# TianyiFranklinWang/MIRROR

Measured on AMD Instinct MI355X. Metric: SSL samples/sec (slide+RNA pairs), higher is better.
Workload: dtype bf16; 1 GPU; BASELINE c2: B=16/GPU x [4096 patch tokens x 1024-d] + [2048 genes], D=512, RNA depth 6 / 8 heads, train mode, local-batch InfoNCE; precision_policy=bf16, per_gpu_batch=16, global_batch=16, parallelism=dp1, grad_bucket_dtype=f32, step_launch=hip_graph

## Files before the change

### include/mirror_hip.h

```cpp
#ifndef MIRROR_HIP_H
#define MIRROR_HIP_H
#include <stdint.h>

#ifdef __cplusplus
extern "C" {
#endif

#define MH_OK 0
#define MH_EINVAL (-1)
#define MH_EUNSUP (-2)
#define MH_EHIP (-3)

#define MH_F32 0
#define MH_BF16 1

#define MH_ACT_NONE 0
#define MH_ACT_RELU 1
#define MH_ACT_GELU 2

typedef void* mh_stream;

const char* mh_last_error(void);
int mh_version(void);
int mh_exp_build(void);
// ... 166 lines not shown
int mh_eye_minus(const float* P, float* T, float d, int BH, int m, mh_stream s);

int mh_seq_finish(void* seq, const float* cls, int B, int N, int add, int D, int dt, mh_stream s);
int mh_seq_finish_bwd(void* dseq, float* dcls, int B, int N, int add, int D, int dt, mh_stream s);
int mh_ppeg_merge(const float* w7, const float* w5, const float* w3, const float* b7, const float* b5,
                  const float* b3, float* merged, float* bsum, int D, mh_stream s);
int mh_ppeg_fwd(const void* x, void* y, const float* merged, const float* bsum, int B, int S, int D,
                int flip, int dt_x, int dt_y, mh_stream s);
int mh_ppeg_wgrad(const void* x, const void* dout, float* dmerged, float* dbsum, int B, int S, int D,
                  int dt_x, int dt_o, mh_stream s);
int mh_ppeg_bwd(const float* x, const float* dy, const float* merged, float* dx, float* dmerged, float* dbsum, int B, int S,
                int D, void* drop_out, float* drop_db, float p, uint64_t seed, uint64_t offset, const uint64_t* dev_base,
                mh_stream s);
int mh_ppeg_grad_scatter(const float* dmerged, const float* dbsum, float* dw7, float* dw5, float* dw3, float* db7,
                         float* db5, float* db3, int D, mh_stream s);

int mh_rank_mask(const float* noise, float* mask, int B, int N, int len_keep, mh_stream s);
int mh_mask_apply_fwd(const void* x, void* y, const float* mask, const float* token, const float* pos, int B, int T, int D,
                      int first, int token_scalar, int dt_x, int dt_y, mh_stream s);
int mh_mask_apply_bwd_dbias_ok(const void* dy, const void* dx, const float* dpos, int D, int dt_dy, int dt_dx);
int mh_mask_apply_bwd(const void* dy, void* dx, const float* mask, float* dtoken, float* dpos, int B, int T, int D,
                      int first, int token_scalar, int dt_dy, int dt_dx, float* dbias, mh_stream s);

typedef struct {
    int32_t B, D, Hh, H;
    float eps, p_drop;
    uint64_t seed, offset;
    const uint64_t* dev_base;
    const void *w_qkv, *w_proj, *w_fc1, *w_fc2;
    const void *wt_qkv, *wt_proj, *wt_fc1, *wt_fc2;
    const float *b_qkv, *b_proj, *b_fc1, *b_fc2;
    const float *g1, *be1, *g2, *be2;
    const float* x;
    float* y;
    float* stats;
    void* qkv;
    float* attn;
    void* o;
    float* x1;
    void* u;
    void* f;
    const float* dy;
    float* dx;
    float *dw_qkv, *dw_proj, *dw_fc1, *dw_fc2, *db_qkv, *db_proj, *db_fc1, *db_fc2, *dg1, *dbe1, *dg2, *dbe2;
    void* scratch;
} mh_rna_block;
// ... 206 lines not shown
```

### mirror_amd/_lib.py

```python
from __future__ import annotations

import ctypes as C
import os

_HERE = os.path.dirname(os.path.abspath(__file__))
LIB_PATH = os.environ.get("MIRROR_HIP_LIB") or os.path.join(_HERE, "lib", "libmirror_hip.so")

MH_F32, MH_BF16 = 0, 1
ACT_NONE, ACT_RELU, ACT_GELU = 0, 1, 2


class GemmEpi(C.Structure):
    _fields_ = [
        ("kind", C.c_int32), ("resid", C.c_void_p),
        ("p", C.c_float), ("seed", C.c_uint64), ("offset", C.c_uint64), ("dev_base", C.c_void_p),
        ("mask", C.c_void_p), ("token", C.c_void_p), ("pos", C.c_void_p),
        ("rows_per_batch", C.c_int32), ("first", C.c_int32),
        ("tgt", C.c_void_p), ("tgt_bs", C.c_int64), ("sq", C.c_void_p),
    ]


class SkinnyWgradItem(C.Structure):
    _fields_ = [("dy", C.c_void_p), ("lddy", C.c_int64), ("x", C.c_void_p), ("ldx", C.c_int64), ("dw", C.c_void_p), ("lddw", C.c_int64),
                ("db", C.c_void_p), ("M", C.c_int32), ("N", C.c_int32), ("K", C.c_int32), ("dt_dy", C.c_int32), ("dt_x", C.c_int32)]
# ... 98 lines not shown
    "mh_eye_minus": [P, P, F, I, I],
    "mh_pinv_chain_prep": [P, P, P, P, P, I, I],
    "mh_pinv_chain_pack": [P, P, I, I],
    "mh_pinv_chain_fwd": [P, P, P, I, I, I, P, P, I],
    "mh_nys_sim2": [P, P, P, P, P, I, I, I, I, F, L, P],
    "mh_nys_dz_dav": [P, P, P, P, P, P, I, I, I],
    "mh_pinv_chain_bwd": [P, P, P, P, P, P, I, I, I],
    "mh_nys_attn1_fwd": [P, P, P, P, P, P, P, I, I, I, I, I, F, I, L, P],
    "mh_nys_attn1_fwd_q8": [P, P, P, P, P, I, I, I, I, I, F, I, P, P, P, F, P, P],
    "mh_nys_attn3_fwd": [P, P, P, P, P, L, P, P, I, I, I, I, I, F, L, P, P],
    "mh_nys_attn1_bwd": [P, P, P, P, P, P, P, P, P, P, P, P, I, I, I, I, I, F, L],
    "mh_nys_attn3_bwd": [P, P, P, P, P, P, P, P, P, P, I, I, I, I, I, F, L],
    "mh_nys_cls_attn": [P, P, P, P, P, P, P, I, I, I, I, I, I, F, L, I, I],
    "mh_seq_finish": [P, P, I, I, I, I, I],
    "mh_seq_finish_bwd": [P, P, I, I, I, I, I],
    "mh_ppeg_merge": [P, P, P, P, P, P, P, P, I],
    "mh_ppeg_fwd": [P, P, P, P, I, I, I, I, I, I],
    "mh_ppeg_wgrad": [P, P, P, P, I, I, I, I, I],
    "mh_ppeg_bwd": [P, P, P, P, P, P, I, I, I, P, P, F, U64, U64, P],
    "mh_ppeg_grad_scatter": [P, P, P, P, P, P, P, P, I],
    "mh_rank_mask": [P, P, I, I, I],
    "mh_mask_apply_fwd": [P, P, P, P, P, I, I, I, I, I, I, I],
    "mh_mask_apply_bwd": [P, P, P, P, P, I, I, I, I, I, I, I, P],
    "mh_headattn_fwd": [P, P, P, I, I, I, I],
    "mh_headattn_bwd": [P, P, P, P, I, I, I, I],
    "mh_add": [P, P, P, L, I, I, I],
    "mh_lm_merge": [P, P, P, L, I, L, I],
    "mh_cast": [P, P, L, I, I],
    "mh_gelu_fwd": [P, P, L, I, I],
    "mh_gelu_bwd": [P, P, P, L, I, I, I],
    "mh_relu_bwd": [P, P, P, L, I, L, L, L, I, I, I],
    "mh_dropout": [P, P, L, F, U64, U64, P, I, I],
    "mh_noise_draws": [P, L, L, U64, U64, P],
    "mh_dropout_add": [P, P, P, L, F, U64, U64, P, I],
    "mh_dropout_lite": [P, P, P, L, F, U64, U64, P, I, I],
    "mh_timestamp": [P],
    "mh_dropout_lite_colsum": [P, P, L, I, F, U64, U64, P, P],
    "mh_colsum": [P, P, L, I, L, I],
    "mh_l2norm_fwd": [P, P, P, I, I, L, F, I, I],
    "mh_l2norm_bwd": [P, P, P, P, I, I, L, F, I, I, I, I],
    "mh_exp_fwd": [P, P, L],
    "mh_exp_bwd": [P, P, P, L, I],
    "mh_reparam_fwd": [P, P, P, P, L],
    "mh_reparam_bwd": [P, P, P, P, P, P, P, L],
    "mh_ce_rows_fwd": [P, L, P, F, I, I, I, F, P, P, P],
    "mh_ce_rows_bwd": [P, L, P, F, P, P, I, F, P, P, I, I, I],
# ... 160 lines not shown
```

### mirror_amd/csrc/elementwise.hip

```cpp
#include "common.h"

#define EW_GRID(n) dim3((unsigned)min((long)mh_cdiv((n), 256), 16384L))
#define EW_LOOP(i, n) for (long i = (long)blockIdx.x * 256 + threadIdx.x; i < (n); i += (long)gridDim.x * 256)

template <typename TA, typename TB, typename TY>
__global__ __launch_bounds__(256) void add_kernel(const TA* a, const TB* b, TY* y, long n) {
    EW_LOOP(i, n) stf(y + i, ldf(a + i) + ldf(b + i));
}
template <typename TX, typename TY>
__global__ __launch_bounds__(256) void cast_kernel(const TX* x, TY* y, long n) {
    EW_LOOP(i, n) stf(y + i, ldf(x + i));
}
template <typename TX, typename TY>
__global__ __launch_bounds__(256) void gelu_fwd_kernel(const TX* x, TY* y, long n) {
    EW_LOOP(i, n) stf(y + i, gelu_f(ldf(x + i)));
}
template <typename TX, typename TDY, typename TDX>
__global__ __launch_bounds__(256) void gelu_bwd_kernel(const TX* x, const TDY* dy, TDX* dx, long n) {
    EW_LOOP(i, n) stf(dx + i, ldf(dy + i) * gelu_grad_f(ldf(x + i)));
}
template <typename TY, typename TDY, typename TDX>
__global__ __launch_bounds__(256) void relu_bwd_kernel(const TY* y, const TDY* dy, TDX* dx, long npb, long y_bs, long dy_bs, long dx_bs) {
    const long b = blockIdx.y;
    EW_LOOP(i, npb) stf(dx + b * dx_bs + i, ldf(y + b * y_bs + i) > 0.f ? ldf(dy + b * dy_bs + i) : 0.f);
// ... 442 lines not shown
extern "C" int mh_colsum(const void* x, float* out, int64_t rows, int cols, int64_t ld, int dt, mh_stream s) {
    if (rows == 0 || cols == 0) return MH_OK;
    if (dt == MH_F32 && cols % 4 == 0 && ld % 4 == 0 && ((uintptr_t)x & 15) == 0 && rows >= 32) {
        dim3 gv(mh_cdiv(cols / 4, 64), (unsigned)min((long)mh_cdiv(rows, 32), 64L));
        hipLaunchKernelGGL(colsum_f32_vec_kernel, gv, dim3(256), 0, (hipStream_t)s, (const float*)x, out, (long)rows, cols, (long)ld);
        MH_LAUNCH_CHECK("mh_colsum");
        return MH_OK;
    }
    if (dt == MH_BF16 && cols % 8 == 0 && ld % 8 == 0 && ((uintptr_t)x & 15) == 0 && rows >= 1024) {
        const int cb = mh_cdiv(cols, 512);
        long nb = max(1L, 512L / cb);
        long band = (mh_cdiv(rows, nb) + 31) / 32 * 32;
        dim3 gv(cb, mh_cdiv(rows, band));
        hipLaunchKernelGGL(colsum_bf16_vec_kernel, gv, dim3(256), 0, (hipStream_t)s, (const bf16_t*)x, out, (long)rows, cols, (long)ld, band);
        MH_LAUNCH_CHECK("mh_colsum");
        return MH_OK;
    }
    dim3 grid(mh_cdiv(cols, 64), mh_cdiv(rows, CS_BAND));
    MH_DISPATCH_DT(dt, T, hipLaunchKernelGGL((colsum_kernel<T>), grid, dim3(256), 0, (hipStream_t)s, (const T*)x, out, (long)rows, cols, (long)ld));
    MH_LAUNCH_CHECK("mh_colsum");
    return MH_OK;
}

__global__ __launch_bounds__(1024) void rank_mask_kernel(const float* __restrict__ noise, float* __restrict__ mask, int N, int P, int len_keep) {
    extern __shared__ __attribute__((aligned(16))) unsigned long long keys[];
    const long b = blockIdx.x;
    const float* nb = noise + b * N;
    for (int j = threadIdx.x; j < P; j += 1024) {
        unsigned long long k = ~0ull;
        if (j < N) {
            unsigned u = __float_as_uint(nb[j]);
            u ^= (u >> 31) ? 0xffffffffu : 0x80000000u;
            k = ((unsigned long long)u << 32) | (unsigned)j;
        }
        keys[j] = k;
    }
    __syncthreads();
    for (int k = 2; k <= P; k <<= 1)
        for (int j = k >> 1; j > 0; j >>= 1) {
            for (int t = threadIdx.x; t < (P >> 1); t += 1024) {
                const int lo = ((t & ~(j - 1)) << 1) | (t & (j - 1)), hi = lo | j;
                const unsigned long long a = keys[lo], c = keys[hi];
                const bool up = (lo & k) == 0;
                if ((a > c) == up) { keys[lo] = c; keys[hi] = a; }
            }
            __syncthreads();
        }
    for (int j = threadIdx.x; j < N; j += 1024) mask[b * N + (unsigned)(keys[j] & 0xffffffffu)] = j >= len_keep ? 1.f : 0.f;
}

extern "C" int mh_rank_mask(const float* noise, float* mask, int B, int N, int len_keep, mh_stream s) {
    MH_REQUIRE(N >= 1 && N <= 16384, "mh_rank_mask: N=%d unsupported (max 16384)", N);
    if (B == 0) return MH_OK;
    int P = 2;
    while (P < N) P <<= 1;
    static const bool big = [] {
        return hipFuncSetAttribute(reinterpret_cast<const void*>(rank_mask_kernel), hipFuncAttributeMaxDynamicSharedMemorySize, 16384 * 8) == hipSuccess;
    }();
    MH_REQUIRE(big || P * 8 <= 65536, "mh_rank_mask: %d bytes of LDS refused", P * 8);
    hipLaunchKernelGGL(rank_mask_kernel, dim3(B), dim3(1024), (size_t)P * sizeof(unsigned long long), (hipStream_t)s, noise, mask, N, P, len_keep);
    MH_LAUNCH_CHECK("mh_rank_mask");
    return MH_OK;
}

template <typename T, typename TY>
__global__ __launch_bounds__(256) void mask_apply_fwd_kernel(const T* x, TY* y, const float* __restrict__ mask,
                                                             const float* __restrict__ token, const float* __restrict__ pos, int B, int Tn,
                                                             int D, int first, int token_scalar) {
    const long total = (long)B * Tn * D;
    EW_LOOP(idx, total) {
        const int c = idx % D;
        const long bt = idx / D;
        const int t = bt % Tn;
        const long b = bt / Tn;
        float v = ldf(x + idx);
        if (t >= first && mask[b * (Tn - first) + (t - first)] != 0.f) v = token[token_scalar ? 0 : c];
        stf(y + idx, v + pos[(long)t * D + c]);
    }
}

typedef float mf_f4 __attribute__((ext_vector_type(4)));
template <typename TX>
__global__ __launch_bounds__(256) void mask_apply_fwd_vec_kernel(const TX* x, float* y, const float* __restrict__ mask,
                                                                 const float* __restrict__ token, const float* __restrict__ pos, int B,
// ... 24 lines not shown
    if (c < D) {
        for (int t = t0 + slice; t < t1; t += 4) {
            float sp = 0.f;
            for (int b = 0; b < B; b++) {
                const long at = ((long)b * Tn + t) * D + c;
                const float g = ldf(dy + at);
                sp += g;
                const bool msk = t >= first && mask[(long)b * (Tn - first) + (t - first)] != 0.f;
                if (msk) st += g;
                stf(dx + at, msk ? 0.f : g);
            }
            dpos[(long)t * D + c] += sp;
        }
    }
    red[slice][lane] = st;
    __syncthreads();
    if (slice == 0 && c < D) {
        const float tot = red[0][lane] + red[1][lane] + red[2][lane] + red[3][lane];
        if (tot != 0.f) atomicAdd(dtoken + (token_scalar ? 0 : c), tot);
    }
}

typedef float mb_f4 __attribute__((ext_vector_type(4)));
template <typename TDX>
__global__ __launch_bounds__(256) void mask_apply_bwd_vec_kernel(const float* dy, TDX* dx, const float* __restrict__ mask,
                                                                 float* __restrict__ dtoken, float* __restrict__ dpos, int B, int Tn, int D,
                                                                 int first, int token_scalar, int band, float* __restrict__ dbias) {
    __shared__ mb_f4 red[4][64];
    __shared__ mb_f4 reda[4][64];
    const int lane = threadIdx.x & 63, wave = threadIdx.x >> 6;
    const int c = blockIdx.x * 256 + 4 * lane;
    const int t0 = blockIdx.y * band, t1 = min(Tn, t0 + band);
    mb_f4 st = {0.f, 0.f, 0.f, 0.f}, sa = {0.f, 0.f, 0.f, 0.f};
    if (c < D) {
        for (int t = t0 + wave; t < t1; t += 4) {
            mb_f4 sp = {0.f, 0.f, 0.f, 0.f};
            for (int b0 = 0; b0 < B; b0 += 8) {
                mb_f4 g[8];
                float mk[8];
#pragma unroll
                for (int u = 0; u < 8; u++)
                    if (b0 + u < B) {
                        g[u] = *reinterpret_cast<const mb_f4*>(dy + ((long)(b0 + u) * Tn + t) * D + c);
                        mk[u] = t >= first ? mask[(long)(b0 + u) * (Tn - first) + (t - first)] : 0.f;
                    }
#pragma unroll
                for (int u = 0; u < 8; u++) {
                    if (b0 + u >= B) break;
                    sp += g[u];
                    const bool msk = mk[u] != 0.f;
                    if (msk) st += g[u];
                    else if constexpr (sizeof(TDX) == 2) {
#pragma unroll
                        for (int e = 0; e < 4; e++) sa[e] += bf2f(f2bf(g[u][e]));
                    } else sa += g[u];
                    if (msk || (const void*)dx != (const void*)dy)
                        st4(dx + ((long)(b0 + u) * Tn + t) * D + c, msk ? (mb_f4){0.f, 0.f, 0.f, 0.f} : g[u]);
                }
            }
            mb_f4* dp = reinterpret_cast<mb_f4*>(dpos + (long)t * D + c);
            *dp = *dp + sp;
        }
    }
    red[wave][lane] = st;
    reda[wave][lane] = sa;
    __syncthreads();
    if (wave == 1 && c < D && dbias) {
        const mb_f4 un = reda[0][lane] + reda[1][lane] + reda[2][lane] + reda[3][lane];
#pragma unroll
        for (int e = 0; e < 4; e++)
            if (un[e] != 0.f) atomicAdd(dbias + c + e, un[e]);
    }
    if (wave == 0 && c < D) {
        const mb_f4 tot = red[0][lane] + red[1][lane] + red[2][lane] + red[3][lane];
        if (token_scalar) {
            const float v = tot[0] + tot[1] + tot[2] + tot[3];
            if (v != 0.f) atomicAdd(dtoken, v);
        } else {
#pragma unroll
// ... 54 lines not shown
    if (T == 0 || D == 0 || B == 0) return MH_OK;
    MH_REQUIRE(!dbias || mh_mask_apply_bwd_dbias_ok(dy, dx, dpos, D, dt_dy, dt_dx),
               "mh_mask_apply_bwd: dbias needs the quad form (f32 dy, D %% 4 == 0, D >= 256, 16-byte aligned operands)");
    if (D == 1) {
#define MAB1_(TDY, TDX) hipLaunchKernelGGL((mask_apply_bwd_d1_kernel<TDY, TDX>), dim3(mh_cdiv(T, 256)), dim3(256), 0, (hipStream_t)s, (const TDY*)dy, (TDX*)dx, mask, dtoken, dpos, B, T, first)
        DISPATCH2(dt_dy, dt_dx, MAB1_)
#undef MAB1_
        MH_LAUNCH_CHECK("mh_mask_apply_bwd");
        return MH_OK;
    }
    if (mh_mask_apply_bwd_dbias_ok(dy, dx, dpos, D, dt_dy, dt_dx)) {
        const int band = 16;
        dim3 gv(mh_cdiv(D, 256), mh_cdiv(T, band));
        if (dt_dx == MH_F32) hipLaunchKernelGGL((mask_apply_bwd_vec_kernel<float>), gv, dim3(256), 0, (hipStream_t)s, (const float*)dy, (float*)dx, mask, dtoken, dpos, B, T, D, first, token_scalar, band, dbias);
        else hipLaunchKernelGGL((mask_apply_bwd_vec_kernel<bf16_t>), gv, dim3(256), 0, (hipStream_t)s, (const float*)dy, (bf16_t*)dx, mask, dtoken, dpos, B, T, D, first, token_scalar, band, dbias);
        MH_LAUNCH_CHECK("mh_mask_apply_bwd");
        return MH_OK;
    }
    dim3 grid(mh_cdiv(D, 64), mh_cdiv(T, MB_BAND));
#define MAB_(TDY, TDX) hipLaunchKernelGGL((mask_apply_bwd_kernel<TDY, TDX>), grid, dim3(256), 0, (hipStream_t)s, (const TDY*)dy, (TDX*)dx, mask, dtoken, dpos, B, T, D, first, token_scalar)
    DISPATCH2(dt_dy, dt_dx, MAB_)
#undef MAB_
    MH_LAUNCH_CHECK("mh_mask_apply_bwd");
    return MH_OK;
}

template <typename T, bool VEC>
__global__ __launch_bounds__(256) void row_scale_kernel(const T* x, const float* __restrict__ sc, T* y, long rows, int D) {
    const int lane = threadIdx.x & 63, wave = threadIdx.x >> 6;
    for (long r = (long)blockIdx.x * 4 + wave; r < rows; r += (long)gridDim.x * 4) {
        const float f = sc[r];
        if (VEC) {
            for (int c = 4 * lane; c < D; c += 256) st4(y + r * D + c, ld4(x + r * D + c) * f);
        } else {
            for (int c = lane; c < D; c += 64) stf(y + r * D + c, ldf(x + r * D + c) * f);
        }
    }
}
extern "C" int mh_row_scale(const void* x, const float* scale, void* y, int64_t rows, int D, int dt, mh_stream s) {
    if (rows == 0 || D == 0) return MH_OK;
    dim3 grid((unsigned)min((long)mh_cdiv(rows, 4), 16384L));
    const bool vec = D % 4 == 0 && mh_quad_ok(x, mh_dt_size(dt)) && mh_quad_ok(y, mh_dt_size(dt));
#define RS_(T)                                                                                                                 \
    if (vec) hipLaunchKernelGGL((row_scale_kernel<T, true>), grid, dim3(256), 0, (hipStream_t)s, (const T*)x, scale, (T*)y, (long)rows, D); \
    else hipLaunchKernelGGL((row_scale_kernel<T, false>), grid, dim3(256), 0, (hipStream_t)s, (const T*)x, scale, (T*)y, (long)rows, D)
    if (dt == MH_F32) { RS_(float); } else { RS_(bf16_t); }
// ... 276 lines not shown
```

### mirror_amd/functional.py

```python
from __future__ import annotations

from dataclasses import dataclass
from typing import List, Optional, Tuple

import os

import torch
from torch.autograd import Function

from . import kernels as K
from ._lib import ACT_NONE, ACT_RELU, MH_BF16, MH_F32

f32, bf16 = torch.float32, torch.bfloat16


@dataclass(frozen=True)
class Precision:
    name: str
    mma: int
    act: torch.dtype
    pinv_mma: int
    fp8_fwd: bool = False


# ... 838 lines not shown

def _mse_bwd_cs(tok, pred, tgt, dp, D):
    if tok is None or not K.mse_masked_bwd_colsum_ok(pred, tgt, dp, D):
        return None
    ws = torch.empty((K.MSE_CS_BLOCKS, D), device=dp.device, dtype=f32)
    tok.offer(dp, ws)
    return ws


def _sq_of(pred, tgt, mask):
    sq = getattr(pred, "_sq", None)
    if sq is None:
        return None
    acc, t0, m0, tv, mv = sq
    if (t0.data_ptr() == tgt.data_ptr() and tuple(t0.shape) == tuple(tgt.shape) and t0.stride() == tgt.stride() and t0._version == tv
            and m0.data_ptr() == mask.data_ptr() and tuple(m0.shape) == tuple(mask.shape) and m0._version == mv):
        return acc
    return None


class EmbedMaskPosFn(Function):

    @staticmethod
    def forward(ctx, h32, h, w, b, mask, token, pos, first, prec):
        wa = shadow(w, prec)
        Bn, T, Kd = h.shape
        N = wa.shape[0]
        out = torch.empty((Bn, T, N), device=h.device, dtype=f32)
        M = Bn * T
        tail = K.linear_fused_tail(M)
        bd = None if b is None else b.detach()
        tok, ps = token.detach().reshape(-1).contiguous(), pos.detach().reshape(T, N).contiguous()
        fork = _tail_fork() if tail else None
        K.linear_fused(h, wa, bd, out, K.epi_maskpos(mask, tok, ps, T, first), m_rows=M - tail)
        if tail and T - tail >= first:
            with _tail_branch(fork, h.device):
                rt = _tail_rows(h[Bn - 1, T - tail:], wa.t(), torch.empty((tail, N), device=h.device, dtype=bf16), bias=bd, mma=prec.mma)
                K.mask_apply_fwd(rt.view(1, tail, N), mask[Bn - 1, T - tail - first:].contiguous(), tok, ps[T - tail:].reshape(-1), 1, tail, N, 0,
                                 False, out=out[Bn - 1:, T - tail:])
        elif tail:
            raise K.MirrorHipError("EmbedMaskPosFn: the tail rows cross the unmasked prefix")
        ctx.save_for_backward(h, wa, w, b, mask)
        ctx.geom = (Bn, T, N, first, token.shape, pos.shape, prec)
        ctx.params = (token, pos)
        return out

    @staticmethod
    def backward(ctx, dy):
        h, wa, w, b, mask = ctx.saved_tensors
        Bn, T, N, first, tshape, pshape, prec = ctx.geom
        dy = dy.contiguous()
        dr = torch.empty(dy.shape, device=dy.device, dtype=prec.act)
        token, pos = ctx.params
        dtok, s_tok = _gbuf_n(token, (N,))
        dpos, s_pos = _gbuf_n(pos, (T * N,))
        db_in = None
        if b is not None and ctx.needs_input_grad[3] and _BIAS_IN_PRODUCER and K.mask_apply_bwd_dbias_ok(dy, dr, dpos, N):
            db_in = _gbuf(b, (N,))
        K.mask_apply_bwd(dy, mask, dtok, dpos, Bn, T, N, first, False, out=dr, dbias=None if db_in is None else db_in[0])
        dtok, dpos = _gret(token, dtok, s_tok), _gret(pos, dpos, s_pos)
        needs = (ctx.needs_input_grad[0], ctx.needs_input_grad[2], ctx.needs_input_grad[3])
        dh, dw, db = _linear_rows_bwd(needs, h, wa, w, b, 0, T, prec, dr, dx_dtype=f32, db_have=db_in)
        return (dh, None, dw, db, None, None if dtok is None else dtok.reshape(tshape), None if dpos is None else dpos.reshape(pshape),
                None, None)


def embed_mask_pos(h, w, b, mask, token, pos, first: int, prec: Precision):
    hb = h if h.dtype == bf16 else getattr(h, "_bf16", None)
    if (hb is not None and prec.act == bf16 and not prec.fp8_fwd and hb.is_contiguous() and tuple(hb.shape) == tuple(h.shape)
            and mask.dtype == f32 and mask.is_contiguous() and hb.shape[1] >= 256 and K.linear_fused_ok(hb, shadow(w, prec))
            and token.numel() == w.shape[0] and pos.numel() == h.shape[1] * w.shape[0]):
        return EmbedMaskPosFn.apply(h, hb, w, b, mask, token, pos, first, prec)
    r = linear(h, w, b, prec=prec)
    return MaskApplyFn.apply(r, mask, token, pos, first, False)


class LayerNormFn(Function):

    @staticmethod
    def forward(ctx, x, gamma, beta, eps, rows, pad, out_dtype, q8_key=None, dual=None, fan_slot=None, res=None, q8_out=None):
        x = x.contiguous()
        Bn, T, D = x.shape
        y = torch.empty((Bn, pad + rows, D), device=x.device, dtype=out_dtype)
        ctx.fan_slot, ctx.res = fan_slot, res
        ctx.drop_site = getattr(x, "_drop_site", None) if (_DROP_IN_LN_BWD and pad == 0 and x.dtype == f32) else None
        if ctx.drop_site is not None and ctx.drop_site.shape != (Bn, T, D):
            ctx.drop_site = None
        if dual is not None:
            mean = torch.empty((Bn * rows,), device=x.device, dtype=f32)
            rstd = torch.empty_like(mean)
            y16 = torch.empty((Bn, rows, D), device=x.device, dtype=bf16)
            K.layernorm_fwd_dual(x, gamma.detach(), beta.detach(), y, y16, mean, rstd, Bn, rows, D, T * D, rows * D, eps)
            dual.append(y16)
            ctx.save_for_backward(x, gamma, mean, rstd, beta)
            ctx.rows, ctx.pad = rows, pad
            return y
        if pad:
# ... 1667 lines not shown
```

### mirror_amd/kernels.py

```python
from __future__ import annotations

import ctypes as C
import functools
import os
from typing import Optional


import torch

from . import _lib
from ._lib import ACT_GELU, ACT_NONE, ACT_RELU, MH_BF16, MH_F32, GemmDesc, MirrorHipError

_DT = {torch.float32: MH_F32, torch.bfloat16: MH_BF16}


def dt(t: torch.Tensor) -> int:
    try:
        return _DT[t.dtype]
    except KeyError:
        raise MirrorHipError(f"unsupported dtype {t.dtype} (f32 / bf16 only)") from None


_raw_stream = getattr(torch._C, "_cuda_getCurrentRawStream", None)

# ... 1184 lines not shown
        out = torch.empty((B, max(N, 0)), device=slot_slide.device, dtype=torch.int64)
    elif out.dtype != torch.int64 or tuple(out.shape) != (B, N) or not out.is_contiguous():
        raise MirrorHipError(f"sample_rows: out must be a contiguous int64 [{B}, {N}] tensor")
    _lib.call("mh_sample_rows", _p(slot_slide), _p(lengths), _p(starts), _p(out), B, N, lengths.numel(), int(seed) & (2 ** 64 - 1), int(offset),
              _p(dev_base), float(slack), stream=_stream())
    return out


def sample_weighted(cdf: torch.Tensor, count: int, seed: int, offset: int, dev_base: Optional[torch.Tensor] = None,
                    out: Optional[torch.Tensor] = None) -> torch.Tensor:
    _chk(cdf, dev_base, out)
    if cdf.dtype != torch.float64 or cdf.dim() != 1 or cdf.numel() == 0 or not cdf.is_contiguous():
        raise MirrorHipError(f"sample_weighted: cdf must be a non-empty contiguous 1-d float64 tensor, got {tuple(cdf.shape)} {cdf.dtype}")
    _draw_base(dev_base, "sample_weighted")
    count = int(count)
    if out is None:
        out = torch.empty((max(count, 0),), device=cdf.device, dtype=torch.int64)
    elif out.dtype != torch.int64 or out.numel() != count or not out.is_contiguous():
        raise MirrorHipError(f"sample_weighted: out must be a contiguous int64 tensor of {count} elements")
    _lib.call("mh_sample_weighted", _p(cdf), cdf.numel(), _p(out), count, int(seed) & (2 ** 64 - 1), int(offset), _p(dev_base), stream=_stream())
    return out


def rank_mask(noise: torch.Tensor, len_keep: int) -> torch.Tensor:
    _chk(noise)
    noise = _contig(noise.float(), "noise")
    B, N = noise.shape
    mask = torch.empty_like(noise)
    _lib.call("mh_rank_mask", _p(noise), _p(mask), B, N, len_keep, stream=_stream())
    return mask


def mask_apply_fwd(x, mask, token, pos, B, T, D, first, token_scalar, out=None) -> None:
    out = x if out is None else out
    _chk(x, mask, token, pos, out)
    assert x.is_contiguous() and x.numel() == B * T * D and mask.numel() == B * (T - first) and pos.numel() == T * D
    assert out.is_contiguous() and out.numel() == x.numel()
    _lib.call("mh_mask_apply_fwd", _p(x), _p(out), _p(mask), _p(token), _p(pos), B, T, D, first, int(token_scalar), dt(x), dt(out),
              stream=_stream())


def mask_apply_bwd_dbias_ok(dy, out, dpos, D) -> bool:
    return bool(_lib.load().mh_mask_apply_bwd_dbias_ok(_p(dy), _p(out), _p(dpos), D, dt(dy), dt(out)))


def mask_apply_bwd(dy, mask, dtoken, dpos, B, T, D, first, token_scalar, out=None, dbias=None) -> None:
    out = dy if out is None else out
    _chk(dy, mask, dtoken, dpos, out)
    assert dy.is_contiguous() and dy.numel() == B * T * D and dpos.numel() == T * D
    assert out.is_contiguous() and out.numel() == dy.numel()
    if dbias is not None:
        _chk(dbias)
        assert dbias.dtype == torch.float32 and dbias.numel() == D and dbias.is_contiguous()
# ... 955 lines not shown
```

### mirror_amd/models/mirror.py

```python
from __future__ import annotations

import logging
import math
import os
from typing import Dict, Optional, Tuple

import numpy as np
import torch
from torch import nn

from .. import functional as Fn
from ..functional import FP32, BF16, POLICIES, Precision
from .._lib import ACT_NONE, MirrorHipError

_logger = logging.getLogger(__name__)
f32 = torch.float32

_DEFAULT_PRECISION: Optional[str] = None

_LM_MASKED = True


def set_precision(name: Optional[str]) -> None:
    global _DEFAULT_PRECISION
# ... 519 lines not shown
        else:
            off0 = st["offset"]
            wsi_mask, mask_ready, (rna_emb, rna_alignment_emb, rna_retention_emb, rna_mask) = run_side()
            self._rna_drop_n[key] = st["offset"] - off0
            wsi_emb = self.wsi_encoder.forward_encoder(wsi_in, wsi_key_padding_mask)
        wsi_full, wsi_retention_target, wsi_cls = Fn.enc_fanout(wsi_emb)
        heads = side
        heads.wait_event(main.record_event())
        wsi_cls.record_stream(heads)
        with torch.cuda.stream(heads):
            Fn.probe("heads_start")
            wsi_alignment_emb = self.wsi_encoder.forward_alignment_head(wsi_cls)
            wsi_score, wsi_mu, wsi_logstd, rna_score, rna_mu, rna_logstd = self.forward_style_clustering(
                wsi_cls, rna_emb, noise.get("wsi_eps"), noise.get("rna_eps"))
            logit_scale = Fn.exp(self.logit_scale)
            Fn.probe("heads_end")
        ag = getattr(self, "_align_gather", None)
        if ag is not None:
            from ..losses.mirror_loss import prefetch_alignment_gather
            with torch.cuda.stream(heads):
                prefetch_alignment_gather(wsi_alignment_emb, rna_alignment_emb, ag[0])
        main.wait_event(mask_ready)
        wsi_mask.record_stream(main)
        Fn.probe("decoder_start")
        wsi_retention_emb, wsi_mask = self.wsi_encoder.forward_retention_head(
            wsi_full, mask_ratio=wsi_mask_ratio, mask=wsi_mask, key_padding_mask=wsi_key_padding_mask,
            target=wsi_retention_target if self.training else None)
        Fn.probe("decoder_end")
        main.wait_stream(side)
        Fn.probe("fwd_joined")
        for t in (rna_emb, rna_alignment_emb, rna_retention_emb, rna_mask, wsi_alignment_emb, wsi_score, wsi_mu, wsi_logstd,
                  rna_score, rna_mu, rna_logstd, logit_scale):
            t.record_stream(main)
        rna_retention_target = rna_emb
        if own_draws:
            Fn.noise_draws_advance()
        return (wsi_alignment_emb, wsi_retention_emb, wsi_retention_target, wsi_mask, wsi_score, wsi_mu, wsi_logstd,
                rna_alignment_emb, rna_retention_emb, rna_retention_target, rna_mask, rna_score, rna_mu, rna_logstd,
                logit_scale)


_ACCEPTED = {
    "wsi_embed_dim", "rna_embed_dim", "embed_dim", "wsi_num_tokens", "wsi_retention_decoder_depth",
    "rna_encoder_depth", "rna_gene_embed", "rna_mlp_ratio", "rna_pos_drop_rate", "rna_proj_drop_rate",
    "rna_attn_drop_rate", "rna_drop_path_rate", "rna_norm_layer", "rna_act_layer", "rna_retention_decoder_depth",
    "init_logit_scale", "style_mlp_hidden_dim", "style_mlp_out_dim", "style_norm_layer", "style_act_layer",
# ... 62 lines not shown
```

Measured before the change: 2204 samples/s.

## Compute masked embed GEMM only on kept rows via keep-index gather/expand

The random-mask ranking kernel now also emits a kept-token index list and a per-token slot map, attached to the mask tensor. When the embed-mask-pos GEMM is large enough, the forward gathers only the kept rows, runs the GEMM on that smaller set, then expands to full length, filling masked positions with the token and adding the positional term. The backward writes gradients only for kept rows, runs the weight and input gradients on the compacted rows, and scatters zeros back for the rest. This skips matmul work on masked rows that would be overwritten, at the cost of extra gather and expand passes and a bf16 round of the GEMM output.

New measurement: 2229 samples/s, median of 6. +1.1%, better.

```diff
diff --git a/include/mirror_hip.h b/include/mirror_hip.h
--- a/include/mirror_hip.h
+++ b/include/mirror_hip.h
@@ -212,6 +212,14 @@
 int mh_mask_apply_bwd(const void* dy, void* dx, const float* mask, float* dtoken, float* dpos, int B, int T, int D,
                       int first, int token_scalar, int dt_dy, int dt_dx, float* dbias, mh_stream s);
 
+int mh_rank_mask_keep(const float* noise, float* mask, int* keep_idx, int* slot, int B, int N, int len_keep, mh_stream s);
+int mh_rows_gather(const void* x, const int* keep_idx, void* out, int B, int T, int K, int first, int keep, mh_stream s);
+int mh_mask_expand_fwd(const void* rc, float* y, const int* slot, const float* token, const float* pos, int B, int T, int D, int first,
+                       int keep, mh_stream s);
+int mh_mask_apply_bwd_keep(const float* dy, void* drc, const int* slot, float* dtoken, float* dpos, int B, int T, int D, int first,
+                           int keep, float* dbias, mh_stream s);
+int mh_rows_expand_zero(const float* dhc, const int* slot, float* dh, int B, int T, int K, int first, int keep, mh_stream s);
+
 typedef struct {
     int32_t B, D, Hh, H;
     float eps, p_drop;
diff --git a/mirror_amd/_lib.py b/mirror_amd/_lib.py
--- a/mirror_amd/_lib.py
+++ b/mirror_amd/_lib.py
@@ -144,6 +144,11 @@
     "mh_rank_mask": [P, P, I, I, I],
     "mh_mask_apply_fwd": [P, P, P, P, P, I, I, I, I, I, I, I],
     "mh_mask_apply_bwd": [P, P, P, P, P, I, I, I, I, I, I, I, P],
+    "mh_rank_mask_keep": [P, P, P, P, I, I, I],
+    "mh_rows_gather": [P, P, P, I, I, I, I, I],
+    "mh_mask_expand_fwd": [P, P, P, P, P, I, I, I, I, I],
+    "mh_mask_apply_bwd_keep": [P, P, P, P, P, I, I, I, I, I, P],
+    "mh_rows_expand_zero": [P, P, P, I, I, I, I, I],
     "mh_headattn_fwd": [P, P, P, I, I, I, I],
     "mh_headattn_bwd": [P, P, P, P, I, I, I, I],
     "mh_add": [P, P, P, L, I, I, I],
diff --git a/mirror_amd/csrc/elementwise.hip b/mirror_amd/csrc/elementwise.hip
--- a/mirror_amd/csrc/elementwise.hip
+++ b/mirror_amd/csrc/elementwise.hip
@@ -488,10 +488,7 @@
     return MH_OK;
 }
 
-__global__ __launch_bounds__(1024) void rank_mask_kernel(const float* __restrict__ noise, float* __restrict__ mask, int N, int P, int len_keep) {
-    extern __shared__ __attribute__((aligned(16))) unsigned long long keys[];
-    const long b = blockIdx.x;
-    const float* nb = noise + b * N;
+__device__ __forceinline__ void rank_sort(unsigned long long* keys, const float* __restrict__ nb, int N, int P) {
     for (int j = threadIdx.x; j < P; j += 1024) {
         unsigned long long k = ~0ull;
         if (j < N) {
@@ -512,7 +509,42 @@
             }
             __syncthreads();
         }
+}
+
+__global__ __launch_bounds__(1024) void rank_mask_kernel(const float* __restrict__ noise, float* __restrict__ mask, int N, int P, int len_keep) {
+    extern __shared__ __attribute__((aligned(16))) unsigned long long keys[];
+    const long b = blockIdx.x;
+    rank_sort(keys, noise + b * N, N, P);
     for (int j = threadIdx.x; j < N; j += 1024) mask[b * N + (unsigned)(keys[j] & 0xffffffffu)] = j >= len_keep ? 1.f : 0.f;
+}
+
+__global__ __launch_bounds__(1024) void rank_mask_keep_kernel(const float* __restrict__ noise, float* __restrict__ mask,
+                                                              int* __restrict__ keep_idx, int* __restrict__ slot, int N, int P, int len_keep) {
+    extern __shared__ __attribute__((aligned(16))) unsigned long long keys[];
+    const long b = blockIdx.x;
+    rank_sort(keys, noise + b * N, N, P);
+    unsigned tok[16];
+#pragma unroll
+    for (int i = 0; i < 16; i++) {
+        const int j = threadIdx.x + 1024 * i;
+        tok[i] = j < N ? (unsigned)(keys[j] & 0xffffffffu) : 0u;
+    }
+    __syncthreads();
+    int* rank = reinterpret_cast<int*>(keys);
+#pragma unroll
+    for (int i = 0; i < 16; i++) {
+        const int j = threadIdx.x + 1024 * i;
+        if (j < N) {
+            rank[tok[i]] = j;
+            if (j < len_keep) keep_idx[b * len_keep + j] = (int)tok[i];
+        }
+    }
+    __syncthreads();
+    for (int t = threadIdx.x; t < N; t += 1024) {
+        const int r = rank[t];
+        mask[b * N + t] = r < len_keep ? 0.f : 1.f;
+        slot[b * N + t] = r < len_keep ? r : -1;
+    }
 }
 
 extern "C" int mh_rank_mask(const float* noise, float* mask, int B, int N, int len_keep, mh_stream s) {
@@ -526,6 +558,22 @@
     MH_REQUIRE(big || P * 8 <= 65536, "mh_rank_mask: %d bytes of LDS refused", P * 8);
     hipLaunchKernelGGL(rank_mask_kernel, dim3(B), dim3(1024), (size_t)P * sizeof(unsigned long long), (hipStream_t)s, noise, mask, N, P, len_keep);
     MH_LAUNCH_CHECK("mh_rank_mask");
+    return MH_OK;
+}
+
+extern "C" int mh_rank_mask_keep(const float* noise, float* mask, int* keep_idx, int* slot, int B, int N, int len_keep, mh_stream s) {
+    MH_REQUIRE(N >= 1 && N <= 16384, "mh_rank_mask_keep: N=%d unsupported (max 16384)", N);
+    MH_REQUIRE(len_keep >= 0 && len_keep <= N && slot && (keep_idx || len_keep == 0), "mh_rank_mask_keep: len_keep=%d of N=%d, or a null map", len_keep, N);
+    if (B == 0) return MH_OK;
+    int P = 2;
+    while (P < N) P <<= 1;
+    static const bool big = [] {
+        return hipFuncSetAttribute(reinterpret_cast<const void*>(rank_mask_keep_kernel), hipFuncAttributeMaxDynamicSharedMemorySize, 16384 * 8) == hipSuccess;
+    }();
+    MH_REQUIRE(big || P * 8 <= 65536, "mh_rank_mask_keep: %d bytes of LDS refused", P * 8);
+    hipLaunchKernelGGL(rank_mask_keep_kernel, dim3(B), dim3(1024), (size_t)P * sizeof(unsigned long long), (hipStream_t)s, noise, mask, keep_idx, slot, N, P,
+                       len_keep);
+    MH_LAUNCH_CHECK("mh_rank_mask_keep");
     return MH_OK;
 }
 
@@ -596,10 +644,11 @@
 }
 
 typedef float mb_f4 __attribute__((ext_vector_type(4)));
-template <typename TDX>
+template <typename TDX, bool KEEP = false>
 __global__ __launch_bounds__(256) void mask_apply_bwd_vec_kernel(const float* dy, TDX* dx, const float* __restrict__ mask,
                                                                  float* __restrict__ dtoken, float* __restrict__ dpos, int B, int Tn, int D,
-                                                                 int first, int token_scalar, int band, float* __restrict__ dbias) {
+                                                                 int first, int token_scalar, int band, float* __restrict__ dbias,
+                                                                 const int* __restrict__ slot = nullptr, int keep = 0) {
     __shared__ mb_f4 red[4][64];
     __shared__ mb_f4 reda[4][64];
     const int lane = threadIdx.x & 63, wave = threadIdx.x >> 6;
@@ -612,11 +661,16 @@
             for (int b0 = 0; b0 < B; b0 += 8) {
                 mb_f4 g[8];
                 float mk[8];
+                int sl[8];
 #pragma unroll
                 for (int u = 0; u < 8; u++)
                     if (b0 + u < B) {
                         g[u] = *reinterpret_cast<const mb_f4*>(dy + ((long)(b0 + u) * Tn + t) * D + c);
-                        mk[u] = t >= first ? mask[(long)(b0 + u) * (Tn - first) + (t - first)] : 0.f;
+                        if constexpr (KEEP) {
+                            const int j = t >= first ? slot[(long)(b0 + u) * (Tn - first) + (t - first)] : t - first;
+                            sl[u] = (j < keep && j >= -first) ? first + j : -1;
+                            mk[u] = (t >= first && j < 0) ? 1.f : 0.f;
+                        } else mk[u] = t >= first ? mask[(long)(b0 + u) * (Tn - first) + (t - first)] : 0.f;
                     }
 #pragma unroll
                 for (int u = 0; u < 8; u++) {
@@ -628,7 +682,9 @@
 #pragma unroll
                         for (int e = 0; e < 4; e++) sa[e] += bf2f(f2bf(g[u][e]));
                     } else sa += g[u];
-                    if (msk || (const void*)dx != (const void*)dy)
+                    if constexpr (KEEP) {
+                        if (!msk && sl[u] >= 0) st4(dx + ((long)(b0 + u) * (first + keep) + sl[u]) * D + c, g[u]);
+                    } else if (msk || (const void*)dx != (const void*)dy)
                         st4(dx + ((long)(b0 + u) * Tn + t) * D + c, msk ? (mb_f4){0.f, 0.f, 0.f, 0.f} : g[u]);
                 }
             }
@@ -729,6 +785,102 @@
     DISPATCH2(dt_dy, dt_dx, MAB_)
 #undef MAB_
     MH_LAUNCH_CHECK("mh_mask_apply_bwd");
+    return MH_OK;
+}
+
+__global__ __launch_bounds__(256) void rows_gather_kernel(const uint4* __restrict__ x, const int* __restrict__ keep_idx, uint4* __restrict__ out,
+                                                          int B, int Tn, int K8, int first, int keep) {
+    const int lane = threadIdx.x & 63, wave = threadIdx.x >> 6;
+    const int Tc = first + keep;
+    const long rows = (long)B * Tc;
+    for (long row = (long)blockIdx.x * 4 + wave; row < rows; row += (long)gridDim.x * 4) {
+        const int r = (int)(row % Tc);
+        const long b = row / Tc;
+        const int t = r < first ? r : first + keep_idx[b * keep + (r - first)];
+        if (t < 0 || t >= Tn) continue;
+        const uint4* src = x + (b * Tn + t) * K8;
+        for (int c = lane; c < K8; c += 64) out[row * K8 + c] = src[c];
+    }
+}
+
+extern "C" int mh_rows_gather(const void* x, const int* keep_idx, void* out, int B, int T, int K, int first, int keep, mh_stream s) {
+    MH_REQUIRE(first >= 0 && keep >= 0 && first + keep <= T && K % 8 == 0 && (((uintptr_t)x | (uintptr_t)out) & 15) == 0 && (keep_idx || keep == 0),
+               "mh_rows_gather: first=%d keep=%d T=%d K=%d (K %% 8 == 0, 16-byte aligned operands)", first, keep, T, K);
+    const long rows = (long)B * (first + keep);
+    if (rows == 0 || K == 0) return MH_OK;
+    hipLaunchKernelGGL(rows_gather_kernel, dim3((unsigned)min((long)mh_cdiv(rows, 4), 16384L)), dim3(256), 0, (hipStream_t)s, (const uint4*)x, keep_idx,
+                       (uint4*)out, B, T, K / 8, first, keep);
+    MH_LAUNCH_CHECK("mh_rows_gather");
+    return MH_OK;
+}
+
+__global__ __launch_bounds__(256) void mask_expand_fwd_kernel(const bf16_t* __restrict__ rc, float* __restrict__ y, const int* __restrict__ slot,
+                                                              const float* __restrict__ token, const float* __restrict__ pos, int B, int Tn, int D,
+                                                              int first, int keep) {
+    const int lane = threadIdx.x & 63, wave = threadIdx.x >> 6;
+    const long rows = (long)B * Tn;
+    for (long row = (long)blockIdx.x * 4 + wave; row < rows; row += (long)gridDim.x * 4) {
+        const int t = (int)(row % Tn);
+        const long b = row / Tn;
+        const int j = t >= first ? slot[b * (Tn - first) + (t - first)] : t - first;
+        const bool masked = (t >= first && j < 0) || j >= keep;
+        const bf16_t* src = rc + (b * (first + keep) + first + j) * D;
+        for (int c = 4 * lane; c < D; c += 256) {
+            const mf_f4 v = masked ? *reinterpret_cast<const mf_f4*>(token + c) : ld4(src + c);
+            *reinterpret_cast<mf_f4*>(y + row * D + c) = v + *reinterpret_cast<const mf_f4*>(pos + (long)t * D + c);
+        }
+    }
+}
+
+extern "C" int mh_mask_expand_fwd(const void* rc, float* y, const int* slot, const float* token, const float* pos, int B, int T, int D, int first,
+                                  int keep, mh_stream s) {
+    MH_REQUIRE(first >= 0 && keep >= 0 && first + keep <= T && D % 4 == 0 && mh_quad_ok(rc, 2) &&
+                   (((uintptr_t)y | (uintptr_t)token | (uintptr_t)pos) & 15) == 0 && (slot || T == first),
+               "mh_mask_expand_fwd: first=%d keep=%d T=%d D=%d (D %% 4 == 0, aligned operands)", first, keep, T, D);
+    const long rows = (long)B * T;
+    if (rows == 0 || D == 0) return MH_OK;
+    hipLaunchKernelGGL(mask_expand_fwd_kernel, dim3((unsigned)min((long)mh_cdiv(rows, 4), 16384L)), dim3(256), 0, (hipStream_t)s, (const bf16_t*)rc, y, slot,
+                       token, pos, B, T, D, first, keep);
+    MH_LAUNCH_CHECK("mh_mask_expand_fwd");
+    return MH_OK;
+}
+
+extern "C" int mh_mask_apply_bwd_keep(const float* dy, void* drc, const int* slot, float* dtoken, float* dpos, int B, int T, int D, int first,
+                                      int keep, float* dbias, mh_stream s) {
+    if (T == 0 || D == 0 || B == 0) return MH_OK;
+    MH_REQUIRE(first >= 0 && keep >= 0 && first + keep <= T && (slot || T == first) && mh_mask_apply_bwd_dbias_ok(dy, drc, dpos, D, MH_F32, MH_BF16),
+               "mh_mask_apply_bwd_keep: first=%d keep=%d T=%d D=%d (the quad form: D %% 4 == 0, D >= 256, 16-byte aligned operands)", first, keep, T, D);
+    const int band = 16;
+    dim3 gv(mh_cdiv(D, 256), mh_cdiv(T, band));
+    hipLaunchKernelGGL((mask_apply_bwd_vec_kernel<bf16_t, true>), gv, dim3(256), 0, (hipStream_t)s, dy, (bf16_t*)drc, (const float*)nullptr, dtoken, dpos,
+                       B, T, D, first, 0, band, dbias, slot, keep);
+    MH_LAUNCH_CHECK("mh_mask_apply_bwd_keep");
+    return MH_OK;
+}
+
+__global__ __launch_bounds__(256) void rows_expand_zero_kernel(const float* __restrict__ dhc, const int* __restrict__ slot, float* __restrict__ dh,
+                                                               int B, int Tn, int K, int first, int keep) {
+    const int lane = threadIdx.x & 63, wave = threadIdx.x >> 6;
+    const long rows = (long)B * Tn;
+    for (long row = (long)blockIdx.x * 4 + wave; row < rows; row += (long)gridDim.x * 4) {
+        const int t = (int)(row % Tn);
+        const long b = row / Tn;
+        const int j = t >= first ? slot[b * (Tn - first) + (t - first)] : t - first;
+        const bool masked = (t >= first && j < 0) || j >= keep;
+        const float* src = dhc + (b * (first + keep) + first + j) * K;
+        for (int c = 4 * lane; c < K; c += 256)
+            *reinterpret_cast<mf_f4*>(dh + row * K + c) = masked ? (mf_f4){0.f, 0.f, 0.f, 0.f} : *reinterpret_cast<const mf_f4*>(src + c);
+    }
+}
+
+extern "C" int mh_rows_expand_zero(const float* dhc, const int* slot, float* dh, int B, int T, int K, int first, int keep, mh_stream s) {
+    MH_REQUIRE(first >= 0 && keep >= 0 && first + keep <= T && K % 4 == 0 && (((uintptr_t)dhc | (uintptr_t)dh) & 15) == 0 && (slot || T == first),
+               "mh_rows_expand_zero: first=%d keep=%d T=%d K=%d (K %% 4 == 0, 16-byte aligned operands)", first, keep, T, K);
+    const long rows = (long)B * T;
+    if (rows == 0 || K == 0) return MH_OK;
+    hipLaunchKernelGGL(rows_expand_zero_kernel, dim3((unsigned)min((long)mh_cdiv(rows, 4), 16384L)), dim3(256), 0, (hipStream_t)s, dhc, slot, dh, B, T, K,
+                       first, keep);
+    MH_LAUNCH_CHECK("mh_rows_expand_zero");
     return MH_OK;
 }
 
diff --git a/mirror_amd/functional.py b/mirror_amd/functional.py
--- a/mirror_amd/functional.py
+++ b/mirror_amd/functional.py
@@ -884,15 +884,25 @@
 class EmbedMaskPosFn(Function):
 
     @staticmethod
-    def forward(ctx, h32, h, w, b, mask, token, pos, first, prec):
+    def forward(ctx, h32, h, w, b, mask, token, pos, first, prec, keepmap=None):
         wa = shadow(w, prec)
         Bn, T, Kd = h.shape
         N = wa.shape[0]
         out = torch.empty((Bn, T, N), device=h.device, dtype=f32)
         M = Bn * T
-        tail = K.linear_fused_tail(M)
         bd = None if b is None else b.detach()
         tok, ps = token.detach().reshape(-1).contiguous(), pos.detach().reshape(T, N).contiguous()
+        ctx.geom = (Bn, T, N, first, token.shape, pos.shape, prec)
+        ctx.params = (token, pos)
+        ctx.keep = None if keepmap is None else keepmap[2]
+        if keepmap is not None:
+            keep_idx, slot, keep = keepmap
+            hc = K.rows_gather(h, keep_idx, first, keep)
+            rc = _gemm_rows(hc, wa.t(), bias=bd, mma=prec.mma, out_dtype=bf16)
+            K.mask_expand_fwd(rc, slot, tok, ps, T, first, keep, out)
+            ctx.save_for_backward(hc, wa, w, b, slot)
+            return out
+        tail = K.linear_fused_tail(M)
         fork = _tail_fork() if tail else None
         K.linear_fused(h, wa, bd, out, K.epi_maskpos(mask, tok, ps, T, first), m_rows=M - tail)
         if tail and T - tail >= first:
@@ -903,28 +913,39 @@
         elif tail:
             raise K.MirrorHipError("EmbedMaskPosFn: the tail rows cross the unmasked prefix")
         ctx.save_for_backward(h, wa, w, b, mask)
-        ctx.geom = (Bn, T, N, first, token.shape, pos.shape, prec)
-        ctx.params = (token, pos)
         return out
 
     @staticmethod
     def backward(ctx, dy):
         h, wa, w, b, mask = ctx.saved_tensors
         Bn, T, N, first, tshape, pshape, prec = ctx.geom
+        keep = ctx.keep
+        Tc = T if keep is None else first + keep
         dy = dy.contiguous()
-        dr = torch.empty(dy.shape, device=dy.device, dtype=prec.act)
+        dr = torch.empty((Bn, Tc, N), device=dy.device, dtype=prec.act)
         token, pos = ctx.params
         dtok, s_tok = _gbuf_n(token, (N,))
         dpos, s_pos = _gbuf_n(pos, (T * N,))
         db_in = None
-        if b is not None and ctx.needs_input_grad[3] and _BIAS_IN_PRODUCER and K.mask_apply_bwd_dbias_ok(dy, dr, dpos, N):
+        quad = K.mask_apply_bwd_dbias_ok(dy, dr, dpos, N)
+        if b is not None and ctx.needs_input_grad[3] and _BIAS_IN_PRODUCER and (quad or keep is not None):
             db_in = _gbuf(b, (N,))
-        K.mask_apply_bwd(dy, mask, dtok, dpos, Bn, T, N, first, False, out=dr, dbias=None if db_in is None else db_in[0])
+        dbias = None if db_in is None else db_in[0]
+        if keep is None:
+            K.mask_apply_bwd(dy, mask, dtok, dpos, Bn, T, N, first, False, out=dr, dbias=dbias)
+        elif quad:
+            K.mask_apply_bwd_keep(dy, mask, dtok, dpos, Bn, T, N, first, keep, out=dr, dbias=dbias)
+        else:
+            dp = zeros((T * N,), dy.device)
+            K.mask_apply_bwd_keep(dy, mask, dtok, dp, Bn, T, N, first, keep, out=dr, dbias=dbias)
+            dpos.add_(dp)
         dtok, dpos = _gret(token, dtok, s_tok), _gret(pos, dpos, s_pos)
         needs = (ctx.needs_input_grad[0], ctx.needs_input_grad[2], ctx.needs_input_grad[3])
-        dh, dw, db = _linear_rows_bwd(needs, h, wa, w, b, 0, T, prec, dr, dx_dtype=f32, db_have=db_in)
+        dh, dw, db = _linear_rows_bwd(needs, h, wa, w, b, 0, Tc, prec, dr, dx_dtype=f32, db_have=db_in)
+        if keep is not None and dh is not None:
+            dh = K.rows_expand_zero(dh, mask, T, first, keep)
         return (dh, None, dw, db, None, None if dtok is None else dtok.reshape(tshape), None if dpos is None else dpos.reshape(pshape),
-                None, None)
+                None, None, None)
 
 
 def embed_mask_pos(h, w, b, mask, token, pos, first: int, prec: Precision):
@@ -932,9 +953,25 @@
     if (hb is not None and prec.act == bf16 and not prec.fp8_fwd and hb.is_contiguous() and tuple(hb.shape) == tuple(h.shape)
             and mask.dtype == f32 and mask.is_contiguous() and hb.shape[1] >= 256 and K.linear_fused_ok(hb, shadow(w, prec))
             and token.numel() == w.shape[0] and pos.numel() == h.shape[1] * w.shape[0]):
-        return EmbedMaskPosFn.apply(h, hb, w, b, mask, token, pos, first, prec)
+        keepmap = _keep_of(mask, hb.shape[0], hb.shape[1] - first)
+        if keepmap is not None and -(-hb.shape[0] * hb.shape[1] // 256) * (w.shape[0] // 256) <= _EMBED_KEEP_TILES:
+            keepmap = None
+        return EmbedMaskPosFn.apply(h, hb, w, b, mask, token, pos, first, prec, keepmap)
     r = linear(h, w, b, prec=prec)
     return MaskApplyFn.apply(r, mask, token, pos, first, False)
+
+
+_EMBED_KEEP_TILES = _CUS
+
+
+def _keep_of(mask, Bn: int, n_tok: int):
+    km = getattr(mask, "_keep", None)
+    if km is None or mask._version != 0 or tuple(mask.shape) != (Bn, n_tok):
+        return None
+    keep_idx, slot, keep = km
+    if tuple(slot.shape) != (Bn, n_tok) or tuple(keep_idx.shape) != (Bn, keep) or slot.device != mask.device:
+        return None
+    return km
 
 
 class LayerNormFn(Function):
diff --git a/mirror_amd/kernels.py b/mirror_amd/kernels.py
--- a/mirror_amd/kernels.py
+++ b/mirror_amd/kernels.py
@@ -1230,13 +1230,73 @@
     return out
 
 
-def rank_mask(noise: torch.Tensor, len_keep: int) -> torch.Tensor:
+def rank_mask(noise: torch.Tensor, len_keep: int, keep_map: bool = True) -> torch.Tensor:
     _chk(noise)
     noise = _contig(noise.float(), "noise")
     B, N = noise.shape
     mask = torch.empty_like(noise)
-    _lib.call("mh_rank_mask", _p(noise), _p(mask), B, N, len_keep, stream=_stream())
+    len_keep = int(len_keep)
+    if not keep_map or not 0 <= len_keep <= N:
+        _lib.call("mh_rank_mask", _p(noise), _p(mask), B, N, len_keep, stream=_stream())
+        return mask
+    keep_idx = torch.empty((B, len_keep), device=noise.device, dtype=torch.int32)
+    slot = torch.empty((B, N), device=noise.device, dtype=torch.int32)
+    _lib.call("mh_rank_mask_keep", _p(noise), _p(mask), _p(keep_idx), _p(slot), B, N, len_keep, stream=_stream())
+    mask._keep = (keep_idx, slot, len_keep)
     return mask
+
+
+def _keep_geom(slot, keep_idx, B, T, first, keep) -> None:
+    for t, shape in ((slot, (B, T - first)), (keep_idx, (B, keep))):
+        if t is not None and not (t.dtype == torch.int32 and t.is_contiguous() and tuple(t.shape) == shape):
+            raise MirrorHipError(f"keep map: expected a contiguous int32 {shape}, got {t.dtype} {tuple(t.shape)}")
+    if not (0 <= first and 0 <= keep and first + keep <= T):
+        raise MirrorHipError(f"keep map: first={first} keep={keep} of T={T}")
+
+
+def rows_gather(x: torch.Tensor, keep_idx: torch.Tensor, first: int, keep: int) -> torch.Tensor:
+    _chk(x, keep_idx)
+    B, T, Kd = x.shape
+    _keep_geom(None, keep_idx, B, T, first, keep)
+    if x.dtype != torch.bfloat16 or not x.is_contiguous():
+        raise MirrorHipError("rows_gather: x must be a contiguous bf16 [B, T, K] tensor")
+    out = torch.empty((B, first + keep, Kd), device=x.device, dtype=torch.bfloat16)
+    _lib.call("mh_rows_gather", _p(x), _p(keep_idx), _p(out), B, T, Kd, first, keep, stream=_stream())
+    return out
+
+
+def mask_expand_fwd(rc: torch.Tensor, slot: torch.Tensor, token: torch.Tensor, pos: torch.Tensor, T: int, first: int, keep: int,
+                    out: torch.Tensor) -> torch.Tensor:
+    _chk(rc, slot, token, pos, out)
+    B, Tc, D = rc.shape
+    _keep_geom(slot, None, B, T, first, keep)
+    if not (rc.dtype == torch.bfloat16 and rc.is_contiguous() and Tc == first + keep and out.dtype == torch.float32 and out.is_contiguous()
+            and tuple(out.shape) == (B, T, D) and token.dtype == pos.dtype == torch.float32 and token.is_contiguous() and pos.is_contiguous()
+            and token.numel() == D and pos.numel() == T * D):
+        raise MirrorHipError("mask_expand_fwd: bad operands")
+    _lib.call("mh_mask_expand_fwd", _p(rc), _p(out), _p(slot), _p(token), _p(pos), B, T, D, first, keep, stream=_stream())
+    return out
+
+
+def mask_apply_bwd_keep(dy, slot, dtoken, dpos, B, T, D, first, keep, out, dbias=None) -> None:
+    _chk(dy, slot, dtoken, dpos, out, dbias)
+    _keep_geom(slot, None, B, T, first, keep)
+    if not (dy.dtype == torch.float32 and dy.is_contiguous() and dy.numel() == B * T * D and out.dtype == torch.bfloat16 and out.is_contiguous()
+            and out.numel() == B * (first + keep) * D and dpos.dtype == dtoken.dtype == torch.float32 and dpos.numel() == T * D
+            and dtoken.numel() == D and (dbias is None or (dbias.dtype == torch.float32 and dbias.numel() == D and dbias.is_contiguous()))):
+        raise MirrorHipError("mask_apply_bwd_keep: bad operands")
+    _lib.call("mh_mask_apply_bwd_keep", _p(dy), _p(out), _p(slot), _p(dtoken), _p(dpos), B, T, D, first, keep, _p(dbias), stream=_stream())
+
+
+def rows_expand_zero(dhc: torch.Tensor, slot: torch.Tensor, T: int, first: int, keep: int) -> torch.Tensor:
+    _chk(dhc, slot)
+    B, Tc, Kd = dhc.shape
+    _keep_geom(slot, None, B, T, first, keep)
+    if not (dhc.dtype == torch.float32 and dhc.is_contiguous() and Tc == first + keep):
+        raise MirrorHipError("rows_expand_zero: dhc must be a contiguous f32 [B, first + keep, K] tensor")
+    dh = torch.empty((B, T, Kd), device=dhc.device, dtype=torch.float32)
+    _lib.call("mh_rows_expand_zero", _p(dhc), _p(slot), _p(dh), B, T, Kd, first, keep, stream=_stream())
+    return dh
 
 
 def mask_apply_fwd(x, mask, token, pos, B, T, D, first, token_scalar, out=None) -> None:
diff --git a/mirror_amd/models/mirror.py b/mirror_amd/models/mirror.py
--- a/mirror_amd/models/mirror.py
+++ b/mirror_amd/models/mirror.py
@@ -565,6 +565,8 @@
                 prefetch_alignment_gather(wsi_alignment_emb, rna_alignment_emb, ag[0])
         main.wait_event(mask_ready)
         wsi_mask.record_stream(main)
+        for t in getattr(wsi_mask, "_keep", ())[:2]:
+            t.record_stream(main)
         Fn.probe("decoder_start")
         wsi_retention_emb, wsi_mask = self.wsi_encoder.forward_retention_head(
             wsi_full, mask_ratio=wsi_mask_ratio, mask=wsi_mask, key_padding_mask=wsi_key_padding_mask,
```
